# dotchen/LAV

Measured on NVIDIA H100. Metric: agent_frames_per_s, higher is better.
Workload: dtype fp16 storage, fp32 accumulate (wgmma f16 / mma.sync f16; saturating stores)

## Files before the change

### lav_b200/csrc/conv_pair_umma.cu

```cuda
#include <stdlib.h>
#include "sm90.cuh"

namespace lavb {
namespace pair {

constexpr int kBlockM = 128, kBlockK = 64;
constexpr int kABytes = kBlockM * kBlockK * 2;
constexpr int kMaxStages = 8;
constexpr int kPairThreads = 288;

struct PairArgs {
  int n, h, w, c, kchunks, dil, tile_w, tile_h, tiles_per_img, num_tiles, stages, post_relu;
  const h16* res;
  const float* bias1; const float* shift2;
  long long* trace; int trace_tiles;
};
#define PAIR_STAMP(slot, i)                                                                                         \
  do {                                                                                                              \
    if (p.trace && threadIdx.x == 0 && (i) < p.trace_tiles)                                                         \
      p.trace[((long long)blockIdx.x * p.trace_tiles + (i)) * 8 + (slot)] = clock64();                              \
  } while (0)

using namespace sm90;

__device__ __forceinline__ uint32_t relu2(uint32_t x) {
  const h162 v = __hmax2(*reinterpret_cast<const h162*>(&x), floats2h162(0.f, 0.f));
  return *reinterpret_cast<const uint32_t*>(&v);
}
__device__ __forceinline__ uint32_t add2(uint32_t x, uint32_t r, bool relu) {
  const h162 a = *reinterpret_cast<const h162*>(&x), b = *reinterpret_cast<const h162*>(&r);
  h162 v = relu ? __hfma2_relu(a, floats2h162(1.f, 1.f), b) : __hadd2(a, b);
#ifndef LAVB_H16_BF16
  const uint32_t hi = 0x7BFF7BFFu, lo = 0xFBFFFBFFu;
  v = __hmin2(v, *reinterpret_cast<const h162*>(&hi));
  if (!relu) v = __hmax2(v, *reinterpret_cast<const h162*>(&lo));
#endif
  return *reinterpret_cast<const uint32_t*>(&v);
}

template <int kC>
__global__ void __launch_bounds__(kPairThreads, kC == 64 ? 2 : 1) conv_pair_umma_kernel(const __grid_constant__ CUtensorMap tmap_a,
                                                                                       const __grid_constant__ CUtensorMap tmap_w1,
                                                                                       const __grid_constant__ CUtensorMap tmap_w2,
                                                                                       const __grid_constant__ CUtensorMap tmap_r,
                                                                                       const __grid_constant__ CUtensorMap tmap_o,
                                                                                       const __grid_constant__ PairArgs p) {
  constexpr int kNC = kC / 64;
  constexpr int kChunks = kC / kBlockK;
  constexpr int kWBytes = kC * kBlockK * 2;
  constexpr int kSlotBytes = kABytes + kWBytes;
  constexpr int kNkb = 3 * kChunks;
  constexpr int kBpf = kSlotBytes / kWBytes;
  constexpr int kOutBytes = kChunks * kABytes;
  static_assert(kNkb % kBpf == 0, "stage 2 fills whole ring slots");
  static_assert(kOutBytes <= kSlotBytes, "the residual / output tile fits one ring slot");
  extern __shared__ uint8_t smem_raw[];
  const uint32_t base = (smem_u32(smem_raw) + 1023u) & ~1023u;
  uint8_t* gen = smem_raw + (base - smem_u32(smem_raw));
  const uint32_t mid = base + p.stages * kSlotBytes;
  constexpr int kMidBytes = 3 * kChunks * kABytes;
  const uint32_t ctrl = mid + kMidBytes;
  const uint32_t full_bar = ctrl, empty_bar = ctrl + 8 * kMaxStages;
  float* ep_b1 = reinterpret_cast<float*>(gen + (ctrl - base) + 16 * kMaxStages);
  float* ep_t2 = ep_b1 + 128;

  const int warp = threadIdx.x >> 5, lane = threadIdx.x & 31;
  if (threadIdx.x == 0) {
    asm volatile("prefetch.tensormap [%0];" ::"l"(reinterpret_cast<uint64_t>(&tmap_a)) : "memory");
    asm volatile("prefetch.tensormap [%0];" ::"l"(reinterpret_cast<uint64_t>(&tmap_w1)) : "memory");
    asm volatile("prefetch.tensormap [%0];" ::"l"(reinterpret_cast<uint64_t>(&tmap_w2)) : "memory");
    asm volatile("prefetch.tensormap [%0];" ::"l"(reinterpret_cast<uint64_t>(&tmap_r)) : "memory");
    asm volatile("prefetch.tensormap [%0];" ::"l"(reinterpret_cast<uint64_t>(&tmap_o)) : "memory");
    for (int s = 0; s < p.stages; ++s) { mbar_init(full_bar + 8 * s, 1); mbar_init(empty_bar + 8 * s, 8); }
    asm volatile("fence.mbarrier_init.release.cluster;" ::: "memory");
  }
  for (int c = threadIdx.x; c < kC; c += blockDim.x) {
    ep_b1[c] = __ldg(p.bias1 + c);
    ep_t2[c] = p.shift2 ? __ldg(p.shift2 + c) : 0.f;
  }
  for (int i = threadIdx.x; i < kMidBytes / 16; i += blockDim.x)
    *reinterpret_cast<uint4*>(gen + (mid - base) + 16 * i) = make_uint4(0u, 0u, 0u, 0u);
  proxy_fence_async();
  __syncthreads();

  if (warp == 8) {
    if (lane == 0) {
      int slot = 0; uint32_t phase = 0;
      for (int tile = blockIdx.x; tile < p.num_tiles; tile += gridDim.x) {
        const int img = tile / p.tiles_per_img, y0 = (tile - img * p.tiles_per_img) * p.tile_h;
        for (int t = 0; t < 3; ++t)
          for (int kc = 0; kc < kChunks; ++kc) {
            mbar_wait(empty_bar + 8 * slot, phase ^ 1);
            const uint32_t sa = base + slot * kSlotBytes;
            mbar_expect_tx(full_bar + 8 * slot, kSlotBytes);
            tma_load_4d(sa, &tmap_a, full_bar + 8 * slot, kc * kBlockK, 0, y0 + (t - 1) * p.dil, img);
            tma_load_2d(sa + kABytes, &tmap_w1, full_bar + 8 * slot, kc * kBlockK, t * kC);
            if (++slot == p.stages) { slot = 0; phase ^= 1; }
          }
        for (int kb0 = 0; kb0 < kNkb; kb0 += kBpf) {
          mbar_wait(empty_bar + 8 * slot, phase ^ 1);
          const uint32_t sa = base + slot * kSlotBytes;
          mbar_expect_tx(full_bar + 8 * slot, kBpf * kWBytes);
          for (int b = 0; b < kBpf; ++b) {
            const int kb = kb0 + b, t = kb / kChunks, kc = kb - t * kChunks;
            tma_load_2d(sa + b * kWBytes, &tmap_w2, full_bar + 8 * slot, kc * kBlockK, t * kC);
          }
          if (++slot == p.stages) { slot = 0; phase ^= 1; }
        }
        mbar_wait(empty_bar + 8 * slot, phase ^ 1);
        if (p.res) {
          mbar_expect_tx(full_bar + 8 * slot, kOutBytes);
          for (int kc = 0; kc < kChunks; ++kc)
            tma_load_4d(base + slot * kSlotBytes + kc * kABytes, &tmap_r, full_bar + 8 * slot, kc * kBlockK, 0, y0, img);
        } else {
          mbar_arrive(full_bar + 8 * slot);
        }
        if (++slot == p.stages) { slot = 0; phase ^= 1; }
      }
    }
    return;
  }

  const int wg = warp >> 2;
  const int d = p.dil;
  const bool relu_out = p.post_relu != 0;
  uint8_t* midp = gen + (mid - base);
  int slot = 0; uint32_t phase = 0;
  int i = 0;
  for (int tile = blockIdx.x; tile < p.num_tiles; tile += gridDim.x, ++i) {
    const int img = tile / p.tiles_per_img, y0 = (tile - img * p.tiles_per_img) * p.tile_h;
    float acc[kC / 2];
    int prev = -1;
    for (int kb = 0; kb < kNkb; ++kb) {
      mbar_wait(full_bar + 8 * slot, phase);
      const uint32_t sa = base + slot * kSlotBytes;
      const uint64_t a_desc = sm90::desc_sw128(sa + wg * (kABytes / 2)), b_desc = sm90::desc_sw128(sa + kABytes);
      sm90::wgmma_fence();
#pragma unroll
      for (int k = 0; k < kBlockK / 16; ++k)
        sm90::wgmma<kC>(acc, a_desc + (uint64_t)(2 * k), b_desc + (uint64_t)(2 * k), (kb | k) ? 1u : 0u);
      sm90::wgmma_commit();
      sm90::wgmma_wait<1>();
      if (prev >= 0 && lane == 0) mbar_arrive(empty_bar + 8 * prev);
      prev = slot;
      if (++slot == p.stages) { slot = 0; phase ^= 1; }
    }
    sm90::wgmma_wait<0>();
    sm90::acc_fence(acc);
    if (lane == 0) mbar_arrive(empty_bar + 8 * prev);
    PAIR_STAMP(0, i);
    sm90::bar_sync(1, 256);
#pragma unroll
    for (int h = 0; h < 2; ++h) {
      const int m = 64 * wg + 16 * (warp & 3) + (lane >> 2) + 8 * h;
      const int px = m % p.tile_w;
      const bool ok0 = px + d < p.tile_w, ok2 = px - d >= 0;
      const int r0 = m + d, r2 = m - d;
#pragma unroll
      for (int cc = 0; cc < kNC; ++cc)
#pragma unroll
        for (int j = 0; j < 8; ++j) {
          const int col = 64 * cc + 8 * j + 2 * (lane & 3);
          const float2 b = *reinterpret_cast<const float2*>(ep_b1 + col);
          const uint32_t v = relu2(pack_h16(acc[32 * cc + 4 * j + 2 * h] + b.x, acc[32 * cc + 4 * j + 2 * h + 1] + b.y));
          uint8_t* blk = midp + cc * kABytes + (col & 7) * 2;
          if (ok0) *reinterpret_cast<uint32_t*>(blk + 0 * kChunks * kABytes + r0 * 128 + ((j ^ (r0 & 7)) << 4)) = v;
          *reinterpret_cast<uint32_t*>(blk + 1 * kChunks * kABytes + m * 128 + ((j ^ (m & 7)) << 4)) = v;
          if (ok2) *reinterpret_cast<uint32_t*>(blk + 2 * kChunks * kABytes + r2 * 128 + ((j ^ (r2 & 7)) << 4)) = v;
        }
    }
    proxy_fence_async();
    sm90::bar_sync(1, 256);
    PAIR_STAMP(1, i);
    prev = -1;
    for (int kb0 = 0; kb0 < kNkb; kb0 += kBpf) {
      mbar_wait(full_bar + 8 * slot, phase);
      const uint32_t sa = base + slot * kSlotBytes;
      sm90::wgmma_fence();
#pragma unroll
      for (int b = 0; b < kBpf; ++b) {
        const uint64_t a_desc = sm90::desc_sw128(mid + (kb0 + b) * kABytes + wg * (kABytes / 2)), b_desc = sm90::desc_sw128(sa + b * kWBytes);
#pragma unroll
        for (int k = 0; k < kBlockK / 16; ++k)
          sm90::wgmma<kC>(acc, a_desc + (uint64_t)(2 * k), b_desc + (uint64_t)(2 * k), (kb0 | b | k) ? 1u : 0u);
      }
      sm90::wgmma_commit();
      sm90::wgmma_wait<1>();
      if (prev >= 0 && lane == 0) mbar_arrive(empty_bar + 8 * prev);
      prev = slot;
      if (++slot == p.stages) { slot = 0; phase ^= 1; }
    }
    sm90::wgmma_wait<0>();
    sm90::acc_fence(acc);
    if (lane == 0) mbar_arrive(empty_bar + 8 * prev);
    PAIR_STAMP(2, i);
    const int out_slot = slot; const uint32_t out_phase = phase;
    if (++slot == p.stages) { slot = 0; phase ^= 1; }
    mbar_wait(full_bar + 8 * out_slot, out_phase);
    uint8_t* outp = gen + out_slot * kSlotBytes;
#pragma unroll
    for (int h = 0; h < 2; ++h) {
      const int m = 64 * wg + 16 * (warp & 3) + (lane >> 2) + 8 * h;
#pragma unroll
      for (int cc = 0; cc < kNC; ++cc)
#pragma unroll
        for (int j = 0; j < 8; ++j) {
          const int col = 64 * cc + 8 * j + 2 * (lane & 3);
          const float2 t = *reinterpret_cast<const float2*>(ep_t2 + col);
          uint32_t* o = reinterpret_cast<uint32_t*>(outp + cc * kABytes + m * 128 + ((j ^ (m & 7)) << 4) + (col & 7) * 2);
          uint32_t v = pack_h16(acc[32 * cc + 4 * j + 2 * h] + t.x, acc[32 * cc + 4 * j + 2 * h + 1] + t.y);
          if (p.res) v = add2(v, *o, relu_out);
          else if (relu_out) v = relu2(v);
          *o = v;
        }
    }
    proxy_fence_async();
    sm90::bar_sync(1, 256);
    if (threadIdx.x == 0) {
      for (int kc = 0; kc < kChunks; ++kc) tma_store_4d(&tmap_o, base + out_slot * kSlotBytes + kc * kABytes, kc * kBlockK, 0, y0, img);
      bulk_commit();
      bulk_wait_read<0>();
      mbar_arrive(empty_bar + 8 * out_slot, 8);
    }
    PAIR_STAMP(3, i);
  }
  if (threadIdx.x == 0) bulk_wait<0>();
}

}
}

using namespace lavb;
using namespace lavb::pair;

static long long* g_pair_trace = nullptr;
static int g_pair_trace_tiles = 0;
extern "C" int lavb_conv_pair_set_trace(void* d_buf, int tiles_per_cta) {
  g_pair_trace = reinterpret_cast<long long*>(d_buf);
  g_pair_trace_tiles = d_buf ? tiles_per_cta : 0;
  return 0;
}

extern "C" int lavb_conv_pair_umma(const lavb_conv_pair_desc* d, void* stream) {
  LAVB_CHECK_ARG(d != nullptr, "conv_pair_umma: null descriptor");
  LAVB_CHECK_ARG(d->c == 64 || d->c == 128, "conv_pair_umma: channels must be 64 or 128 (got %d)", d->c);
  LAVB_CHECK_ARG(d->w == 32 || d->w == 64 || d->w == 128, "conv_pair_umma: image width must be 32, 64 or 128 (a tile is made of full rows)");
  LAVB_CHECK_ARG(d->dil >= 1 && d->dil < d->w, "conv_pair_umma: dilation must be in [1, width)");
  LAVB_CHECK_ARG(d->n >= 0 && d->h >= 1, "conv_pair_umma: bad shape");
  LAVB_CHECK_ARG(d->w1 && d->w2 && d->bias1 && d->in && d->out, "conv_pair_umma: null operand");
  {
    const size_t bytes = (size_t)d->n * d->h * d->w * d->c * 2;
    const auto overlap = [&](const void* x) {
      const char *o = static_cast<const char*>(d->out), *q = static_cast<const char*>(x);
      return x && o < q + bytes && q < o + bytes;
    };
    LAVB_CHECK_ARG(!overlap(d->in) && !overlap(d->res), "conv_pair_umma: out must not overlap in or res");
  }
  if (d->n == 0) return 0;
  auto encode = get_encode();
  LAVB_CHECK_ARG(encode != nullptr, "conv_pair_umma: cuTensorMapEncodeTiled not available from the driver");
  PairArgs a;
  memset(&a, 0, sizeof(a));
  a.n = d->n; a.h = d->h; a.w = d->w; a.c = d->c; a.kchunks = d->c / kBlockK; a.dil = d->dil;
  a.tile_w = d->w; a.tile_h = kBlockM / d->w;
  a.tiles_per_img = ceil_div(d->h, a.tile_h);
  a.num_tiles = d->n * a.tiles_per_img;
  a.post_relu = d->post_relu;
  a.res = reinterpret_cast<const h16*>(d->res);
  a.bias1 = d->bias1; a.shift2 = d->shift2;
  a.trace = g_pair_trace; a.trace_tiles = g_pair_trace_tiles;
  const int slot_bytes = kABytes + d->c * kBlockK * 2;
  const int mid_bytes = 3 * a.kchunks * kABytes;
  const int ctrl_bytes = 1024  + 16 * kMaxStages + 2 * 128 * (int)sizeof(float);
  const bool two = d->c == 64;
  const int smem_cap = two ? 113 * 1024 : 227 * 1024;
  a.stages = min(kMaxStages, (smem_cap - mid_bytes - ctrl_bytes) / slot_bytes);
  const int smem = a.stages * slot_bytes + mid_bytes + ctrl_bytes;
  CUtensorMap tmap_a, tmap_w1, tmap_w2, tmap_r, tmap_o;
  const auto encode_act = [&](CUtensorMap* m, const void* ptr) {
    cuuint64_t dims[4] = {(cuuint64_t)d->c, (cuuint64_t)d->w, (cuuint64_t)d->h, (cuuint64_t)d->n};
    cuuint64_t strides[3] = {(cuuint64_t)d->c * 2, (cuuint64_t)d->w * d->c * 2, (cuuint64_t)d->h * d->w * d->c * 2};
    cuuint32_t box[4] = {(cuuint32_t)kBlockK, (cuuint32_t)a.tile_w, (cuuint32_t)a.tile_h, 1};
    cuuint32_t estr[4] = {1, 1, 1, 1};
    return encode(m, LAVB_TMAP_H16, 4, const_cast<void*>(ptr), dims, strides, box, estr, CU_TENSOR_MAP_INTERLEAVE_NONE,
                  CU_TENSOR_MAP_SWIZZLE_128B, CU_TENSOR_MAP_L2_PROMOTION_L2_256B, CU_TENSOR_MAP_FLOAT_OOB_FILL_NONE);
  };
  CUresult r = encode_act(&tmap_a, d->in);
  LAVB_CHECK_ARG(r == CUDA_SUCCESS, "conv_pair_umma: cuTensorMapEncodeTiled(in) failed with %d", (int)r);
  r = encode_act(&tmap_r, d->res ? d->res : d->in);
  LAVB_CHECK_ARG(r == CUDA_SUCCESS, "conv_pair_umma: cuTensorMapEncodeTiled(res) failed with %d", (int)r);
  r = encode_act(&tmap_o, d->out);
  LAVB_CHECK_ARG(r == CUDA_SUCCESS, "conv_pair_umma: cuTensorMapEncodeTiled(out) failed with %d", (int)r);
  for (int which = 0; which < 2; ++which) {
    cuuint64_t dims[2] = {(cuuint64_t)d->c, (cuuint64_t)3 * d->c};
    cuuint64_t strides[1] = {(cuuint64_t)d->c * 2};
    cuuint32_t box[2] = {(cuuint32_t)kBlockK, (cuuint32_t)d->c};
    cuuint32_t estr[2] = {1, 1};
    CUresult r = encode(which ? &tmap_w2 : &tmap_w1, LAVB_TMAP_H16, 2, const_cast<void*>(which ? d->w2 : d->w1), dims,
                        strides, box, estr, CU_TENSOR_MAP_INTERLEAVE_NONE, CU_TENSOR_MAP_SWIZZLE_128B, CU_TENSOR_MAP_L2_PROMOTION_L2_256B,
                        CU_TENSOR_MAP_FLOAT_OOB_FILL_NONE);
    LAVB_CHECK_ARG(r == CUDA_SUCCESS, "conv_pair_umma: cuTensorMapEncodeTiled(W%d) failed with %d", which + 1, (int)r);
  }
  if (two) {
    LAVB_CUDA_OK(ensure_dyn_smem((const void*)conv_pair_umma_kernel<64>, smem_cap));
    conv_pair_umma_kernel<64><<<min(a.num_tiles, 2 * kNumSMs), kPairThreads, smem, (cudaStream_t)stream>>>(tmap_a, tmap_w1, tmap_w2, tmap_r, tmap_o, a);
  } else {
    LAVB_CUDA_OK(ensure_dyn_smem((const void*)conv_pair_umma_kernel<128>, smem_cap));
    conv_pair_umma_kernel<128><<<min(a.num_tiles, kNumSMs), kPairThreads, smem, (cudaStream_t)stream>>>(tmap_a, tmap_w1, tmap_w2, tmap_r, tmap_o, a);
  }
  LAVB_LAUNCH_OK();
  return 0;
}
```

### lav_b200/csrc/sm90.cuh

```cuda
#pragma once
#include <cuda.h>
#include <cudaTypedefs.h>
#include "common.cuh"

namespace lavb {
namespace sm90 {

__device__ __forceinline__ uint32_t smem_u32(const void* p) { return (uint32_t)__cvta_generic_to_shared(p); }

__device__ __forceinline__ void proxy_fence_async() { asm volatile("fence.proxy.async.shared::cta;" ::: "memory"); }
__device__ __forceinline__ void bar_sync(int id, int threads) { asm volatile("bar.sync %0, %1;" ::"r"(id), "r"(threads) : "memory"); }

__device__ __forceinline__ void mbar_init(uint32_t bar, uint32_t count) {
  asm volatile("mbarrier.init.shared::cta.b64 [%0], %1;" ::"r"(bar), "r"(count));
}
__device__ __forceinline__ void mbar_expect_tx(uint32_t bar, uint32_t bytes) {
  asm volatile("mbarrier.arrive.expect_tx.shared::cta.b64 _, [%0], %1;" ::"r"(bar), "r"(bytes) : "memory");
}
__device__ __forceinline__ void mbar_arrive(uint32_t bar) {
  asm volatile("mbarrier.arrive.shared::cta.b64 _, [%0];" ::"r"(bar) : "memory");
}
__device__ __forceinline__ void mbar_wait(uint32_t bar, uint32_t parity) {
  uint32_t done;
  do {
    asm volatile(
        "{\n\t.reg .pred p;\n\t"
        "mbarrier.try_wait.parity.shared::cta.b64 p, [%1], %2;\n\t"
        "selp.u32 %0, 1, 0, p;\n\t}"
        : "=r"(done) : "r"(bar), "r"(parity) : "memory");
  } while (!done);
}
__device__ __forceinline__ void tma_load_4d(uint32_t dst, const CUtensorMap* map, uint32_t bar, int c0, int c1, int c2, int c3) {
  asm volatile(
      "cp.async.bulk.tensor.4d.shared::cluster.global.mbarrier::complete_tx::bytes [%0], [%1, {%3, %4, %5, %6}], [%2];"
      ::"r"(dst), "l"(reinterpret_cast<uint64_t>(map)), "r"(bar), "r"(c0), "r"(c1), "r"(c2), "r"(c3) : "memory");
}
__device__ __forceinline__ void tma_load_2d(uint32_t dst, const CUtensorMap* map, uint32_t bar, int c0, int c1) {
  asm volatile(
      "cp.async.bulk.tensor.2d.shared::cluster.global.mbarrier::complete_tx::bytes [%0], [%1, {%3, %4}], [%2];"
      ::"r"(dst), "l"(reinterpret_cast<uint64_t>(map)), "r"(bar), "r"(c0), "r"(c1) : "memory");
}
__device__ __forceinline__ void mbar_arrive(uint32_t bar, uint32_t count) {
  asm volatile("mbarrier.arrive.shared::cta.b64 _, [%0], %1;" ::"r"(bar), "r"(count) : "memory");
}

__device__ __forceinline__ void tma_store_4d(const CUtensorMap* map, uint32_t src, int c0, int c1, int c2, int c3) {
  asm volatile("cp.async.bulk.tensor.4d.global.shared::cta.bulk_group [%0, {%2, %3, %4, %5}], [%1];"
               ::"l"(reinterpret_cast<uint64_t>(map)), "r"(src), "r"(c0), "r"(c1), "r"(c2), "r"(c3) : "memory");
}
__device__ __forceinline__ void bulk_commit() { asm volatile("cp.async.bulk.commit_group;" ::: "memory"); }
template <int N> __device__ __forceinline__ void bulk_wait_read() { asm volatile("cp.async.bulk.wait_group.read %0;" ::"n"(N) : "memory"); }
template <int N> __device__ __forceinline__ void bulk_wait() { asm volatile("cp.async.bulk.wait_group %0;" ::"n"(N) : "memory"); }

inline PFN_cuTensorMapEncodeTiled_v12000 get_encode() {
  static PFN_cuTensorMapEncodeTiled_v12000 fn = nullptr;
  if (!fn) {
    void* p = nullptr;
    cudaDriverEntryPointQueryResult q;
    if (cudaGetDriverEntryPoint("cuTensorMapEncodeTiled", &p, cudaEnableDefault, &q) == cudaSuccess && q == cudaDriverEntryPointSuccess)
      fn = reinterpret_cast<PFN_cuTensorMapEncodeTiled_v12000>(p);
  }
  return fn;
}

__device__ __forceinline__ uint64_t desc_sw128(uint32_t saddr) {
  const uint32_t lo = ((saddr & 0x3FFFFu) >> 4) | (1u << 16);
  const uint32_t hi = (1024u >> 4) | (1u << 30);
  return (uint64_t)lo | ((uint64_t)hi << 32);
}

__device__ __forceinline__ void wgmma_fence() { asm volatile("wgmma.fence.sync.aligned;" ::: "memory"); }
__device__ __forceinline__ void wgmma_commit() { asm volatile("wgmma.commit_group.sync.aligned;" ::: "memory"); }
template <int N> __device__ __forceinline__ void wgmma_wait() { asm volatile("wgmma.wait_group.sync.aligned %0;" ::"n"(N) : "memory"); }
template <int N> __device__ __forceinline__ void acc_fence(float (&d)[N]) {
#pragma unroll
  for (int i = 0; i < N; ++i) asm volatile("" : "+f"(d[i])::"memory");
}

template <int N> __device__ void wgmma(float (&d)[N / 2], uint64_t a, uint64_t b, uint32_t accumulate);

#define LAVB_WG_R0 "%0, %1, %2, %3, %4, %5, %6, %7, %8, %9, %10, %11, %12, %13, %14, %15"
#define LAVB_WG_R1 "%16, %17, %18, %19, %20, %21, %22, %23, %24, %25, %26, %27, %28, %29, %30, %31"
#define LAVB_WG_R2 "%32, %33, %34, %35, %36, %37, %38, %39, %40, %41, %42, %43, %44, %45, %46, %47"
#define LAVB_WG_R3 "%48, %49, %50, %51, %52, %53, %54, %55, %56, %57, %58, %59, %60, %61, %62, %63"
#define LAVB_WG_R4 "%64, %65, %66, %67, %68, %69, %70, %71, %72, %73, %74, %75, %76, %77, %78, %79"
#define LAVB_WG_R5 "%80, %81, %82, %83, %84, %85, %86, %87, %88, %89, %90, %91, %92, %93, %94, %95"
#define LAVB_WG_R6 "%96, %97, %98, %99, %100, %101, %102, %103, %104, %105, %106, %107, %108, %109, %110, %111"
#define LAVB_WG_R7 "%112, %113, %114, %115, %116, %117, %118, %119, %120, %121, %122, %123, %124, %125, %126, %127"
#define LAVB_WG_D4(i) "+f"(d[i]), "+f"(d[i + 1]), "+f"(d[i + 2]), "+f"(d[i + 3])
#define LAVB_WG_D16(i) LAVB_WG_D4(i), LAVB_WG_D4(i + 4), LAVB_WG_D4(i + 8), LAVB_WG_D4(i + 12)
#define LAVB_WGMMA(N, REGS, IA, IB, IP, ...)                                                                         \
  template <> __device__ __forceinline__ void wgmma<N>(float (&d)[N / 2], uint64_t a, uint64_t b, uint32_t accumulate) { \
    asm volatile(                                                                                                      \
        "{\n\t.reg .pred p;\n\t"                                                                                       \
        "setp.ne.b32 p, %" #IP ", 0;\n\t"                                                                              \
        "wgmma.mma_async.sync.aligned.m64n" #N "k16.f32." LAVB_H16_PTX "." LAVB_H16_PTX " "                            \
        "{" REGS "}, %" #IA ", %" #IB ", p, 1, 1, 0, 0;\n\t}"                                                          \
        : __VA_ARGS__                                                                                                  \
        : "l"(a), "l"(b), "r"(accumulate));                                                                            \
  }
LAVB_WGMMA(32, LAVB_WG_R0, 16, 17, 18, LAVB_WG_D16(0))
LAVB_WGMMA(64, LAVB_WG_R0 ", " LAVB_WG_R1, 32, 33, 34, LAVB_WG_D16(0), LAVB_WG_D16(16))
LAVB_WGMMA(96, LAVB_WG_R0 ", " LAVB_WG_R1 ", " LAVB_WG_R2, 48, 49, 50, LAVB_WG_D16(0), LAVB_WG_D16(16), LAVB_WG_D16(32))
LAVB_WGMMA(128, LAVB_WG_R0 ", " LAVB_WG_R1 ", " LAVB_WG_R2 ", " LAVB_WG_R3, 64, 65, 66,
           LAVB_WG_D16(0), LAVB_WG_D16(16), LAVB_WG_D16(32), LAVB_WG_D16(48))
LAVB_WGMMA(160, LAVB_WG_R0 ", " LAVB_WG_R1 ", " LAVB_WG_R2 ", " LAVB_WG_R3 ", " LAVB_WG_R4, 80, 81, 82,
           LAVB_WG_D16(0), LAVB_WG_D16(16), LAVB_WG_D16(32), LAVB_WG_D16(48), LAVB_WG_D16(64))
LAVB_WGMMA(192, LAVB_WG_R0 ", " LAVB_WG_R1 ", " LAVB_WG_R2 ", " LAVB_WG_R3 ", " LAVB_WG_R4 ", " LAVB_WG_R5, 96, 97, 98,
           LAVB_WG_D16(0), LAVB_WG_D16(16), LAVB_WG_D16(32), LAVB_WG_D16(48), LAVB_WG_D16(64), LAVB_WG_D16(80))
LAVB_WGMMA(224, LAVB_WG_R0 ", " LAVB_WG_R1 ", " LAVB_WG_R2 ", " LAVB_WG_R3 ", " LAVB_WG_R4 ", " LAVB_WG_R5 ", " LAVB_WG_R6,
           112, 113, 114, LAVB_WG_D16(0), LAVB_WG_D16(16), LAVB_WG_D16(32), LAVB_WG_D16(48), LAVB_WG_D16(64), LAVB_WG_D16(80),
           LAVB_WG_D16(96))
LAVB_WGMMA(256, LAVB_WG_R0 ", " LAVB_WG_R1 ", " LAVB_WG_R2 ", " LAVB_WG_R3 ", " LAVB_WG_R4 ", " LAVB_WG_R5 ", " LAVB_WG_R6 ", " LAVB_WG_R7,
           128, 129, 130, LAVB_WG_D16(0), LAVB_WG_D16(16), LAVB_WG_D16(32), LAVB_WG_D16(48), LAVB_WG_D16(64), LAVB_WG_D16(80),
           LAVB_WG_D16(96), LAVB_WG_D16(112))
#undef LAVB_WGMMA
#undef LAVB_WG_D16
#undef LAVB_WG_D4
#undef LAVB_WG_R0
#undef LAVB_WG_R1
#undef LAVB_WG_R2
#undef LAVB_WG_R3
#undef LAVB_WG_R4
#undef LAVB_WG_R5
#undef LAVB_WG_R6
#undef LAVB_WG_R7

}
}
```

Before: 1962.

## Overlap next tile's stage-1 GEMM with epilogue in fused conv pair kernel

Restructures the fused two-conv kernel so consumers issue the next tile's stage-1 wgmmas while still running the current tile's stage-2 epilogue, using a second accumulator set. For C=64 both weight sets stay resident in shared memory instead of being streamed per tile. The output/residual tile moves to its own double-buffered region with separate barriers so TMA stores overlap. A full producer warpgroup with setmaxnreg register rebalancing is added, and C=64 drops from two CTAs per SM to one. Register pressure is higher, and the lost second CTA on C=64 reduces inter-CTA overlap.

```diff
diff --git a/lav_b200/csrc/conv_pair_umma.cu b/lav_b200/csrc/conv_pair_umma.cu
--- a/lav_b200/csrc/conv_pair_umma.cu
+++ b/lav_b200/csrc/conv_pair_umma.cu
@@ -7,10 +7,35 @@
 constexpr int kBlockM = 128, kBlockK = 64;
 constexpr int kABytes = kBlockM * kBlockK * 2;
 constexpr int kMaxStages = 8;
-constexpr int kPairThreads = 288;
+constexpr int kPairThreads = 384;
+constexpr int kProducerRegs = 40, kConsumerRegs = 232;
+constexpr int kSmemCap = 227 * 1024;
+
+template <int kC>
+struct Cfg {
+  static constexpr bool kResident = kC == 64;
+  static constexpr int kNC = kC / 64;
+  static constexpr int kChunks = kC / kBlockK;
+  static constexpr int kWBytes = kC * kBlockK * 2;
+  static constexpr int kSlotBytes = kABytes + (kResident ? 0 : kWBytes);
+  static constexpr int kNkb = 3 * kChunks;
+  static constexpr int kBpf = kSlotBytes / kWBytes;
+  static constexpr int kOutBytes = kChunks * kABytes;
+  static constexpr int kMidBytes = 3 * kChunks * kABytes;
+  static constexpr int kResBytes = kResident ? 2 * kNkb * kWBytes : 0;
+  static constexpr int kPieces = 2 * kNC;
+  static constexpr int kAhead = kNkb - kPieces;
+  static constexpr int kOutBufs = kC == 64 ? 2 : 1;
+  static constexpr int kCtrlBytes = 1024  + 16 * kMaxStages + 64 + 2 * 128 * (int)sizeof(float);
+  static constexpr int kFixedBytes = kOutBufs * kOutBytes + kMidBytes + kResBytes + kCtrlBytes;
+  static constexpr int kStages = (kSmemCap - kFixedBytes) / kSlotBytes < kMaxStages ? (kSmemCap - kFixedBytes) / kSlotBytes : kMaxStages;
+  static constexpr int kSmemBytes = kStages * kSlotBytes + kFixedBytes;
+  static_assert(kResident || kNkb % kBpf == 0, "stage 2 fills whole ring slots");
+  static_assert(kAhead >= 1 && kStages >= kAhead + 1, "the look-ahead keeps kAhead + 1 stage-1 K-blocks in the ring");
+};
 
 struct PairArgs {
-  int n, h, w, c, kchunks, dil, tile_w, tile_h, tiles_per_img, num_tiles, stages, post_relu;
+  int n, h, w, c, kchunks, dil, tile_w, tile_h, tiles_per_img, num_tiles, post_relu;
   const h16* res;
   const float* bias1; const float* shift2;
   long long* trace; int trace_tiles;
@@ -38,31 +63,220 @@
   return *reinterpret_cast<const uint32_t*>(&v);
 }
 
-template <int kC>
-__global__ void __launch_bounds__(kPairThreads, kC == 64 ? 2 : 1) conv_pair_umma_kernel(const __grid_constant__ CUtensorMap tmap_a,
-                                                                                       const __grid_constant__ CUtensorMap tmap_w1,
-                                                                                       const __grid_constant__ CUtensorMap tmap_w2,
-                                                                                       const __grid_constant__ CUtensorMap tmap_r,
-                                                                                       const __grid_constant__ CUtensorMap tmap_o,
-                                                                                       const __grid_constant__ PairArgs p) {
-  constexpr int kNC = kC / 64;
-  constexpr int kChunks = kC / kBlockK;
-  constexpr int kWBytes = kC * kBlockK * 2;
-  constexpr int kSlotBytes = kABytes + kWBytes;
-  constexpr int kNkb = 3 * kChunks;
-  constexpr int kBpf = kSlotBytes / kWBytes;
-  constexpr int kOutBytes = kChunks * kABytes;
-  static_assert(kNkb % kBpf == 0, "stage 2 fills whole ring slots");
-  static_assert(kOutBytes <= kSlotBytes, "the residual / output tile fits one ring slot");
+struct Smem {
+  uint32_t ring, out, mid, wres;
+  uint32_t full_bar, empty_bar;
+  uint32_t out_full, out_empty;
+  uint32_t w_full;
+  uint8_t* gen;
+  float *ep_b1, *ep_t2;
+};
+
+struct RingPos {
+  int slot = 0; uint32_t phase = 0;
+  template <int kStages> __device__ __forceinline__ void next() { if (++slot == kStages) { slot = 0; phase ^= 1; } }
+};
+
+struct Consumer {
+  RingPos head; int tail = 0;
+  int wg, warp, lane;
+  template <int kStages> __device__ __forceinline__ void release(const Smem& s) {
+    if (lane == 0) mbar_arrive(s.empty_bar + 8 * tail);
+    if (++tail == kStages) tail = 0;
+  }
+};
+
+template <int kC>
+__device__ __forceinline__ void fill_stage1(const Smem& s, RingPos& pos, const CUtensorMap* tmap_a, const CUtensorMap* tmap_w1,
+                                            const PairArgs& p, int tile) {
+  using C = Cfg<kC>;
+  const int img = tile / p.tiles_per_img, y0 = (tile - img * p.tiles_per_img) * p.tile_h;
+  for (int t = 0; t < 3; ++t)
+    for (int kc = 0; kc < C::kChunks; ++kc) {
+      mbar_wait(s.empty_bar + 8 * pos.slot, pos.phase ^ 1);
+      const uint32_t sa = s.ring + pos.slot * C::kSlotBytes, bar = s.full_bar + 8 * pos.slot;
+      mbar_expect_tx(bar, C::kSlotBytes);
+      tma_load_4d(sa, tmap_a, bar, kc * kBlockK, 0, y0 + (t - 1) * p.dil, img);
+      if (!C::kResident) tma_load_2d(sa + kABytes, tmap_w1, bar, kc * kBlockK, t * kC);
+      pos.template next<C::kStages>();
+    }
+}
+
+template <int kC>
+__device__ __forceinline__ void issue_stage1(float (&acc1)[kC / 2], const Smem& s, Consumer& c, int kb) {
+  using C = Cfg<kC>;
+  mbar_wait(s.full_bar + 8 * c.head.slot, c.head.phase);
+  const uint32_t sa = s.ring + c.head.slot * C::kSlotBytes;
+  const uint64_t a_desc = desc_sw128(sa + c.wg * (kABytes / 2));
+  const uint64_t b_desc = desc_sw128(C::kResident ? s.wres + kb * C::kWBytes : sa + kABytes);
+  wgmma_fence();
+#pragma unroll
+  for (int k = 0; k < kBlockK / 16; ++k)
+    wgmma<kC>(acc1, a_desc + (uint64_t)(2 * k), b_desc + (uint64_t)(2 * k), (kb | k) ? 1u : 0u);
+  wgmma_commit();
+  c.head.template next<C::kStages>();
+}
+
+template <int kC>
+__device__ __forceinline__ void stage1(float (&acc1)[kC / 2], const Smem& s, Consumer& c) {
+  using C = Cfg<kC>;
+#pragma unroll
+  for (int kb = 0; kb < C::kNkb; ++kb) {
+    issue_stage1<kC>(acc1, s, c, kb);
+    wgmma_wait<1>();
+    if (kb) c.template release<C::kStages>(s);
+  }
+  wgmma_wait<0>();
+  acc_fence(acc1);
+  c.template release<C::kStages>(s);
+}
+
+template <int kC, bool kLook>
+__device__ __forceinline__ void finish_tile(float (&acc1)[kC / 2], float (&acc2)[kC / 2], const Smem& s, Consumer& c,
+                                            const CUtensorMap* tmap_o, const PairArgs& p, int tile, int i) {
+  using C = Cfg<kC>;
+  const int wg = c.wg, warp = c.warp, lane = c.lane, d = p.dil;
+  const bool relu_out = p.post_relu != 0;
+  const int img = tile / p.tiles_per_img, y0 = (tile - img * p.tiles_per_img) * p.tile_h;
+  uint8_t* midp = s.gen + (s.mid - s.ring);
+  bar_sync(1, 256);
+#pragma unroll
+  for (int h = 0; h < 2; ++h) {
+    const int m = 64 * wg + 16 * (warp & 3) + (lane >> 2) + 8 * h;
+    const int px = m % p.tile_w;
+    const bool ok0 = px + d < p.tile_w, ok2 = px - d >= 0;
+    const int r0 = m + d, r2 = m - d;
+#pragma unroll
+    for (int cc = 0; cc < C::kNC; ++cc) {
+      float2 b1v[8];
+#pragma unroll
+      for (int j = 0; j < 8; ++j) b1v[j] = *reinterpret_cast<const float2*>(s.ep_b1 + 64 * cc + 8 * j + 2 * (lane & 3));
+#pragma unroll
+      for (int j = 0; j < 8; ++j) {
+        const int col = 64 * cc + 8 * j + 2 * (lane & 3);
+        const float2 b = b1v[j];
+        const uint32_t v = relu2(pack_h16(acc1[32 * cc + 4 * j + 2 * h] + b.x, acc1[32 * cc + 4 * j + 2 * h + 1] + b.y));
+        uint8_t* blk = midp + cc * kABytes + (col & 7) * 2;
+        if (ok0) *reinterpret_cast<uint32_t*>(blk + 0 * C::kChunks * kABytes + r0 * 128 + ((j ^ (r0 & 7)) << 4)) = v;
+        *reinterpret_cast<uint32_t*>(blk + 1 * C::kChunks * kABytes + m * 128 + ((j ^ (m & 7)) << 4)) = v;
+        if (ok2) *reinterpret_cast<uint32_t*>(blk + 2 * C::kChunks * kABytes + r2 * 128 + ((j ^ (r2 & 7)) << 4)) = v;
+      }
+    }
+  }
+  proxy_fence_async();
+  bar_sync(1, 256);
+  PAIR_STAMP(1, i);
+  if (C::kResident) {
+    wgmma_fence();
+#pragma unroll
+    for (int kb = 0; kb < C::kNkb; ++kb) {
+      const uint64_t a_desc = desc_sw128(s.mid + kb * kABytes + wg * (kABytes / 2));
+      const uint64_t b_desc = desc_sw128(s.wres + (C::kNkb + kb) * C::kWBytes);
+#pragma unroll
+      for (int k = 0; k < kBlockK / 16; ++k)
+        wgmma<kC>(acc2, a_desc + (uint64_t)(2 * k), b_desc + (uint64_t)(2 * k), (kb | k) ? 1u : 0u);
+    }
+    wgmma_commit();
+  } else {
+#pragma unroll
+    for (int kb0 = 0; kb0 < C::kNkb; kb0 += C::kBpf) {
+      mbar_wait(s.full_bar + 8 * c.head.slot, c.head.phase);
+      const uint32_t sa = s.ring + c.head.slot * C::kSlotBytes;
+      wgmma_fence();
+#pragma unroll
+      for (int b = 0; b < C::kBpf; ++b) {
+        const uint64_t a_desc = desc_sw128(s.mid + (kb0 + b) * kABytes + wg * (kABytes / 2)), b_desc = desc_sw128(sa + b * C::kWBytes);
+#pragma unroll
+        for (int k = 0; k < kBlockK / 16; ++k)
+          wgmma<kC>(acc2, a_desc + (uint64_t)(2 * k), b_desc + (uint64_t)(2 * k), (kb0 | b | k) ? 1u : 0u);
+      }
+      wgmma_commit();
+      c.head.template next<C::kStages>();
+      wgmma_wait<1>();
+      if (kb0) c.template release<C::kStages>(s);
+    }
+  }
+  wgmma_wait<0>();
+  acc_fence(acc2);
+  if (!C::kResident) c.template release<C::kStages>(s);
+  PAIR_STAMP(2, i);
+  if (kLook) {
+#pragma unroll
+    for (int kb = 0; kb < C::kAhead; ++kb) issue_stage1<kC>(acc1, s, c, kb);
+    PAIR_STAMP(4, i);
+  }
+  const int ob = i % C::kOutBufs;
+  mbar_wait(s.out_full + 8 * ob, (i / C::kOutBufs) & 1);
+  uint8_t* outp = s.gen + (s.out - s.ring) + ob * C::kOutBytes;
+#pragma unroll
+  for (int h = 0; h < 2; ++h) {
+    const int m = 64 * wg + 16 * (warp & 3) + (lane >> 2) + 8 * h;
+#pragma unroll
+    for (int cc = 0; cc < C::kNC; ++cc) {
+      uint8_t* orow = outp + cc * kABytes + m * 128 + 4 * (lane & 3);
+      float2 t2v[8];
+      uint32_t r[8];
+#pragma unroll
+      for (int j = 0; j < 8; ++j) t2v[j] = *reinterpret_cast<const float2*>(s.ep_t2 + 64 * cc + 8 * j + 2 * (lane & 3));
+      if (p.res) {
+#pragma unroll
+        for (int j = 0; j < 8; ++j) r[j] = *reinterpret_cast<const uint32_t*>(orow + ((j ^ (m & 7)) << 4));
+      }
+#pragma unroll
+      for (int j = 0; j < 8; ++j) {
+        const float2 t = t2v[j];
+        uint32_t v = pack_h16(acc2[32 * cc + 4 * j + 2 * h] + t.x, acc2[32 * cc + 4 * j + 2 * h + 1] + t.y);
+        if (p.res) v = add2(v, r[j], relu_out);
+        else if (relu_out) v = relu2(v);
+        *reinterpret_cast<uint32_t*>(orow + ((j ^ (m & 7)) << 4)) = v;
+      }
+      if (kLook) {
+        issue_stage1<kC>(acc1, s, c, C::kAhead + h * C::kNC + cc);
+        wgmma_wait<C::kAhead>();
+        c.template release<C::kStages>(s);
+      }
+    }
+  }
+  if (kLook) PAIR_STAMP(5, i);
+  proxy_fence_async();
+  bar_sync(1, 256);
+  if (threadIdx.x == 0) {
+    for (int kc = 0; kc < C::kChunks; ++kc)
+      tma_store_4d(tmap_o, s.out + ob * C::kOutBytes + kc * kABytes, kc * kBlockK, 0, y0, img);
+    bulk_commit();
+    bulk_wait_read<C::kOutBufs - 1>();
+    if (i >= C::kOutBufs - 1) mbar_arrive(s.out_empty + 8 * ((i - (C::kOutBufs - 1)) % C::kOutBufs));
+  }
+  PAIR_STAMP(3, i);
+  if (kLook) {
+    wgmma_wait<0>();
+    acc_fence(acc1);
+#pragma unroll
+    for (int kb = 0; kb < C::kAhead; ++kb) c.template release<C::kStages>(s);
+    PAIR_STAMP(0, i + 1);
+  }
+}
+
+template <int kC>
+__global__ void __launch_bounds__(kPairThreads, 1) conv_pair_umma_kernel(const __grid_constant__ CUtensorMap tmap_a,
+                                                                         const __grid_constant__ CUtensorMap tmap_w1,
+                                                                         const __grid_constant__ CUtensorMap tmap_w2,
+                                                                         const __grid_constant__ CUtensorMap tmap_r,
+                                                                         const __grid_constant__ CUtensorMap tmap_o,
+                                                                         const __grid_constant__ PairArgs p) {
+  using C = Cfg<kC>;
   extern __shared__ uint8_t smem_raw[];
-  const uint32_t base = (smem_u32(smem_raw) + 1023u) & ~1023u;
-  uint8_t* gen = smem_raw + (base - smem_u32(smem_raw));
-  const uint32_t mid = base + p.stages * kSlotBytes;
-  constexpr int kMidBytes = 3 * kChunks * kABytes;
-  const uint32_t ctrl = mid + kMidBytes;
-  const uint32_t full_bar = ctrl, empty_bar = ctrl + 8 * kMaxStages;
-  float* ep_b1 = reinterpret_cast<float*>(gen + (ctrl - base) + 16 * kMaxStages);
-  float* ep_t2 = ep_b1 + 128;
+  Smem s;
+  s.ring = (smem_u32(smem_raw) + 1023u) & ~1023u;
+  s.gen = smem_raw + (s.ring - smem_u32(smem_raw));
+  s.out = s.ring + C::kStages * C::kSlotBytes;
+  s.mid = s.out + C::kOutBufs * C::kOutBytes;
+  s.wres = s.mid + C::kMidBytes;
+  const uint32_t ctrl = s.wres + C::kResBytes;
+  s.full_bar = ctrl; s.empty_bar = ctrl + 8 * kMaxStages;
+  s.out_full = ctrl + 16 * kMaxStages; s.out_empty = s.out_full + 16; s.w_full = s.out_full + 32;
+  s.ep_b1 = reinterpret_cast<float*>(s.gen + (ctrl - s.ring) + 16 * kMaxStages + 64);
+  s.ep_t2 = s.ep_b1 + 128;
 
   const int warp = threadIdx.x >> 5, lane = threadIdx.x & 31;
   if (threadIdx.x == 0) {
@@ -71,159 +285,74 @@
     asm volatile("prefetch.tensormap [%0];" ::"l"(reinterpret_cast<uint64_t>(&tmap_w2)) : "memory");
     asm volatile("prefetch.tensormap [%0];" ::"l"(reinterpret_cast<uint64_t>(&tmap_r)) : "memory");
     asm volatile("prefetch.tensormap [%0];" ::"l"(reinterpret_cast<uint64_t>(&tmap_o)) : "memory");
-    for (int s = 0; s < p.stages; ++s) { mbar_init(full_bar + 8 * s, 1); mbar_init(empty_bar + 8 * s, 8); }
+    for (int i = 0; i < C::kStages; ++i) { mbar_init(s.full_bar + 8 * i, 1); mbar_init(s.empty_bar + 8 * i, 8); }
+    for (int i = 0; i < C::kOutBufs; ++i) { mbar_init(s.out_full + 8 * i, 1); mbar_init(s.out_empty + 8 * i, 1); }
+    mbar_init(s.w_full, 1);
     asm volatile("fence.mbarrier_init.release.cluster;" ::: "memory");
   }
   for (int c = threadIdx.x; c < kC; c += blockDim.x) {
-    ep_b1[c] = __ldg(p.bias1 + c);
-    ep_t2[c] = p.shift2 ? __ldg(p.shift2 + c) : 0.f;
-  }
-  for (int i = threadIdx.x; i < kMidBytes / 16; i += blockDim.x)
-    *reinterpret_cast<uint4*>(gen + (mid - base) + 16 * i) = make_uint4(0u, 0u, 0u, 0u);
+    s.ep_b1[c] = __ldg(p.bias1 + c);
+    s.ep_t2[c] = p.shift2 ? __ldg(p.shift2 + c) : 0.f;
+  }
+  for (int i = threadIdx.x; i < C::kMidBytes / 16; i += blockDim.x)
+    *reinterpret_cast<uint4*>(s.gen + (s.mid - s.ring) + 16 * i) = make_uint4(0u, 0u, 0u, 0u);
   proxy_fence_async();
   __syncthreads();
 
-  if (warp == 8) {
-    if (lane == 0) {
-      int slot = 0; uint32_t phase = 0;
-      for (int tile = blockIdx.x; tile < p.num_tiles; tile += gridDim.x) {
+  const int first = blockIdx.x, step = gridDim.x;
+  if (warp >= 8) {
+    reg_dec<kProducerRegs>();
+    if (warp == 8 && lane == 0 && first < p.num_tiles) {
+      RingPos pos;
+      if (C::kResident) {
+        mbar_expect_tx(s.w_full, C::kResBytes);
+        for (int kb = 0; kb < 2 * C::kNkb; ++kb) {
+          const int t = (kb % C::kNkb) / C::kChunks, kc = kb % C::kChunks;
+          tma_load_2d(s.wres + kb * C::kWBytes, kb < C::kNkb ? &tmap_w1 : &tmap_w2, s.w_full, kc * kBlockK, t * kC);
+        }
+      }
+      fill_stage1<kC>(s, pos, &tmap_a, &tmap_w1, p, first);
+      int i = 0;
+      for (int tile = first; tile < p.num_tiles; tile += step, ++i) {
         const int img = tile / p.tiles_per_img, y0 = (tile - img * p.tiles_per_img) * p.tile_h;
-        for (int t = 0; t < 3; ++t)
-          for (int kc = 0; kc < kChunks; ++kc) {
-            mbar_wait(empty_bar + 8 * slot, phase ^ 1);
-            const uint32_t sa = base + slot * kSlotBytes;
-            mbar_expect_tx(full_bar + 8 * slot, kSlotBytes);
-            tma_load_4d(sa, &tmap_a, full_bar + 8 * slot, kc * kBlockK, 0, y0 + (t - 1) * p.dil, img);
-            tma_load_2d(sa + kABytes, &tmap_w1, full_bar + 8 * slot, kc * kBlockK, t * kC);
-            if (++slot == p.stages) { slot = 0; phase ^= 1; }
+        if (!C::kResident)
+          for (int kb0 = 0; kb0 < C::kNkb; kb0 += C::kBpf) {
+            mbar_wait(s.empty_bar + 8 * pos.slot, pos.phase ^ 1);
+            const uint32_t sa = s.ring + pos.slot * C::kSlotBytes, bar = s.full_bar + 8 * pos.slot;
+            mbar_expect_tx(bar, C::kBpf * C::kWBytes);
+            for (int b = 0; b < C::kBpf; ++b) {
+              const int kb = kb0 + b, t = kb / C::kChunks, kc = kb - t * C::kChunks;
+              tma_load_2d(sa + b * C::kWBytes, &tmap_w2, bar, kc * kBlockK, t * kC);
+            }
+            pos.template next<C::kStages>();
           }
-        for (int kb0 = 0; kb0 < kNkb; kb0 += kBpf) {
-          mbar_wait(empty_bar + 8 * slot, phase ^ 1);
-          const uint32_t sa = base + slot * kSlotBytes;
-          mbar_expect_tx(full_bar + 8 * slot, kBpf * kWBytes);
-          for (int b = 0; b < kBpf; ++b) {
-            const int kb = kb0 + b, t = kb / kChunks, kc = kb - t * kChunks;
-            tma_load_2d(sa + b * kWBytes, &tmap_w2, full_bar + 8 * slot, kc * kBlockK, t * kC);
-          }
-          if (++slot == p.stages) { slot = 0; phase ^= 1; }
+        const int ob = i % C::kOutBufs;
+        const uint32_t out_bar = s.out_full + 8 * ob;
+        mbar_wait(s.out_empty + 8 * ob, ((i / C::kOutBufs) & 1) ^ 1);
+        if (p.res) {
+          mbar_expect_tx(out_bar, C::kOutBytes);
+          for (int kc = 0; kc < C::kChunks; ++kc)
+            tma_load_4d(s.out + ob * C::kOutBytes + kc * kABytes, &tmap_r, out_bar, kc * kBlockK, 0, y0, img);
+        } else {
+          mbar_arrive(out_bar);
         }
-        mbar_wait(empty_bar + 8 * slot, phase ^ 1);
-        if (p.res) {
-          mbar_expect_tx(full_bar + 8 * slot, kOutBytes);
-          for (int kc = 0; kc < kChunks; ++kc)
-            tma_load_4d(base + slot * kSlotBytes + kc * kABytes, &tmap_r, full_bar + 8 * slot, kc * kBlockK, 0, y0, img);
-        } else {
-          mbar_arrive(full_bar + 8 * slot);
-        }
-        if (++slot == p.stages) { slot = 0; phase ^= 1; }
+        if (tile + step < p.num_tiles) fill_stage1<kC>(s, pos, &tmap_a, &tmap_w1, p, tile + step);
       }
     }
     return;
   }
 
-  const int wg = warp >> 2;
-  const int d = p.dil;
-  const bool relu_out = p.post_relu != 0;
-  uint8_t* midp = gen + (mid - base);
-  int slot = 0; uint32_t phase = 0;
-  int i = 0;
-  for (int tile = blockIdx.x; tile < p.num_tiles; tile += gridDim.x, ++i) {
-    const int img = tile / p.tiles_per_img, y0 = (tile - img * p.tiles_per_img) * p.tile_h;
-    float acc[kC / 2];
-    int prev = -1;
-    for (int kb = 0; kb < kNkb; ++kb) {
-      mbar_wait(full_bar + 8 * slot, phase);
-      const uint32_t sa = base + slot * kSlotBytes;
-      const uint64_t a_desc = sm90::desc_sw128(sa + wg * (kABytes / 2)), b_desc = sm90::desc_sw128(sa + kABytes);
-      sm90::wgmma_fence();
-#pragma unroll
-      for (int k = 0; k < kBlockK / 16; ++k)
-        sm90::wgmma<kC>(acc, a_desc + (uint64_t)(2 * k), b_desc + (uint64_t)(2 * k), (kb | k) ? 1u : 0u);
-      sm90::wgmma_commit();
-      sm90::wgmma_wait<1>();
-      if (prev >= 0 && lane == 0) mbar_arrive(empty_bar + 8 * prev);
-      prev = slot;
-      if (++slot == p.stages) { slot = 0; phase ^= 1; }
-    }
-    sm90::wgmma_wait<0>();
-    sm90::acc_fence(acc);
-    if (lane == 0) mbar_arrive(empty_bar + 8 * prev);
-    PAIR_STAMP(0, i);
-    sm90::bar_sync(1, 256);
-#pragma unroll
-    for (int h = 0; h < 2; ++h) {
-      const int m = 64 * wg + 16 * (warp & 3) + (lane >> 2) + 8 * h;
-      const int px = m % p.tile_w;
-      const bool ok0 = px + d < p.tile_w, ok2 = px - d >= 0;
-      const int r0 = m + d, r2 = m - d;
-#pragma unroll
-      for (int cc = 0; cc < kNC; ++cc)
-#pragma unroll
-        for (int j = 0; j < 8; ++j) {
-          const int col = 64 * cc + 8 * j + 2 * (lane & 3);
-          const float2 b = *reinterpret_cast<const float2*>(ep_b1 + col);
-          const uint32_t v = relu2(pack_h16(acc[32 * cc + 4 * j + 2 * h] + b.x, acc[32 * cc + 4 * j + 2 * h + 1] + b.y));
-          uint8_t* blk = midp + cc * kABytes + (col & 7) * 2;
-          if (ok0) *reinterpret_cast<uint32_t*>(blk + 0 * kChunks * kABytes + r0 * 128 + ((j ^ (r0 & 7)) << 4)) = v;
-          *reinterpret_cast<uint32_t*>(blk + 1 * kChunks * kABytes + m * 128 + ((j ^ (m & 7)) << 4)) = v;
-          if (ok2) *reinterpret_cast<uint32_t*>(blk + 2 * kChunks * kABytes + r2 * 128 + ((j ^ (r2 & 7)) << 4)) = v;
-        }
-    }
-    proxy_fence_async();
-    sm90::bar_sync(1, 256);
-    PAIR_STAMP(1, i);
-    prev = -1;
-    for (int kb0 = 0; kb0 < kNkb; kb0 += kBpf) {
-      mbar_wait(full_bar + 8 * slot, phase);
-      const uint32_t sa = base + slot * kSlotBytes;
-      sm90::wgmma_fence();
-#pragma unroll
-      for (int b = 0; b < kBpf; ++b) {
-        const uint64_t a_desc = sm90::desc_sw128(mid + (kb0 + b) * kABytes + wg * (kABytes / 2)), b_desc = sm90::desc_sw128(sa + b * kWBytes);
-#pragma unroll
-        for (int k = 0; k < kBlockK / 16; ++k)
-          sm90::wgmma<kC>(acc, a_desc + (uint64_t)(2 * k), b_desc + (uint64_t)(2 * k), (kb0 | b | k) ? 1u : 0u);
-      }
-      sm90::wgmma_commit();
-      sm90::wgmma_wait<1>();
-      if (prev >= 0 && lane == 0) mbar_arrive(empty_bar + 8 * prev);
-      prev = slot;
-      if (++slot == p.stages) { slot = 0; phase ^= 1; }
-    }
-    sm90::wgmma_wait<0>();
-    sm90::acc_fence(acc);
-    if (lane == 0) mbar_arrive(empty_bar + 8 * prev);
-    PAIR_STAMP(2, i);
-    const int out_slot = slot; const uint32_t out_phase = phase;
-    if (++slot == p.stages) { slot = 0; phase ^= 1; }
-    mbar_wait(full_bar + 8 * out_slot, out_phase);
-    uint8_t* outp = gen + out_slot * kSlotBytes;
-#pragma unroll
-    for (int h = 0; h < 2; ++h) {
-      const int m = 64 * wg + 16 * (warp & 3) + (lane >> 2) + 8 * h;
-#pragma unroll
-      for (int cc = 0; cc < kNC; ++cc)
-#pragma unroll
-        for (int j = 0; j < 8; ++j) {
-          const int col = 64 * cc + 8 * j + 2 * (lane & 3);
-          const float2 t = *reinterpret_cast<const float2*>(ep_t2 + col);
-          uint32_t* o = reinterpret_cast<uint32_t*>(outp + cc * kABytes + m * 128 + ((j ^ (m & 7)) << 4) + (col & 7) * 2);
-          uint32_t v = pack_h16(acc[32 * cc + 4 * j + 2 * h] + t.x, acc[32 * cc + 4 * j + 2 * h + 1] + t.y);
-          if (p.res) v = add2(v, *o, relu_out);
-          else if (relu_out) v = relu2(v);
-          *o = v;
-        }
-    }
-    proxy_fence_async();
-    sm90::bar_sync(1, 256);
-    if (threadIdx.x == 0) {
-      for (int kc = 0; kc < kChunks; ++kc) tma_store_4d(&tmap_o, base + out_slot * kSlotBytes + kc * kABytes, kc * kBlockK, 0, y0, img);
-      bulk_commit();
-      bulk_wait_read<0>();
-      mbar_arrive(empty_bar + 8 * out_slot, 8);
-    }
-    PAIR_STAMP(3, i);
-  }
+  reg_inc<kConsumerRegs>();
+  if (first >= p.num_tiles) return;
+  Consumer c;
+  c.wg = warp >> 2; c.warp = warp; c.lane = lane;
+  float acc1[kC / 2], acc2[kC / 2];
+  if (C::kResident) mbar_wait(s.w_full, 0);
+  stage1<kC>(acc1, s, c);
+  PAIR_STAMP(0, 0);
+  int tile = first, i = 0;
+  for (; tile + step < p.num_tiles; tile += step, ++i) finish_tile<kC, true>(acc1, acc2, s, c, &tmap_o, p, tile, i);
+  finish_tile<kC, false>(acc1, acc2, s, c, &tmap_o, p, tile, i);
   if (threadIdx.x == 0) bulk_wait<0>();
 }
 
@@ -239,6 +368,15 @@
   g_pair_trace = reinterpret_cast<long long*>(d_buf);
   g_pair_trace_tiles = d_buf ? tiles_per_cta : 0;
   return 0;
+}
+
+template <int kC>
+static cudaError_t launch_pair(const CUtensorMap& tmap_a, const CUtensorMap& tmap_w1, const CUtensorMap& tmap_w2, const CUtensorMap& tmap_r,
+                               const CUtensorMap& tmap_o, const PairArgs& a, cudaStream_t stream) {
+  const cudaError_t e = ensure_dyn_smem((const void*)conv_pair_umma_kernel<kC>, Cfg<kC>::kSmemBytes);
+  if (e != cudaSuccess) return e;
+  conv_pair_umma_kernel<kC><<<min(a.num_tiles, kNumSMs), kPairThreads, Cfg<kC>::kSmemBytes, stream>>>(tmap_a, tmap_w1, tmap_w2, tmap_r, tmap_o, a);
+  return cudaSuccess;
 }
 
 extern "C" int lavb_conv_pair_umma(const lavb_conv_pair_desc* d, void* stream) {
@@ -269,13 +407,6 @@
   a.res = reinterpret_cast<const h16*>(d->res);
   a.bias1 = d->bias1; a.shift2 = d->shift2;
   a.trace = g_pair_trace; a.trace_tiles = g_pair_trace_tiles;
-  const int slot_bytes = kABytes + d->c * kBlockK * 2;
-  const int mid_bytes = 3 * a.kchunks * kABytes;
-  const int ctrl_bytes = 1024  + 16 * kMaxStages + 2 * 128 * (int)sizeof(float);
-  const bool two = d->c == 64;
-  const int smem_cap = two ? 113 * 1024 : 227 * 1024;
-  a.stages = min(kMaxStages, (smem_cap - mid_bytes - ctrl_bytes) / slot_bytes);
-  const int smem = a.stages * slot_bytes + mid_bytes + ctrl_bytes;
   CUtensorMap tmap_a, tmap_w1, tmap_w2, tmap_r, tmap_o;
   const auto encode_act = [&](CUtensorMap* m, const void* ptr) {
     cuuint64_t dims[4] = {(cuuint64_t)d->c, (cuuint64_t)d->w, (cuuint64_t)d->h, (cuuint64_t)d->n};
@@ -301,13 +432,8 @@
                         CU_TENSOR_MAP_FLOAT_OOB_FILL_NONE);
     LAVB_CHECK_ARG(r == CUDA_SUCCESS, "conv_pair_umma: cuTensorMapEncodeTiled(W%d) failed with %d", which + 1, (int)r);
   }
-  if (two) {
-    LAVB_CUDA_OK(ensure_dyn_smem((const void*)conv_pair_umma_kernel<64>, smem_cap));
-    conv_pair_umma_kernel<64><<<min(a.num_tiles, 2 * kNumSMs), kPairThreads, smem, (cudaStream_t)stream>>>(tmap_a, tmap_w1, tmap_w2, tmap_r, tmap_o, a);
-  } else {
-    LAVB_CUDA_OK(ensure_dyn_smem((const void*)conv_pair_umma_kernel<128>, smem_cap));
-    conv_pair_umma_kernel<128><<<min(a.num_tiles, kNumSMs), kPairThreads, smem, (cudaStream_t)stream>>>(tmap_a, tmap_w1, tmap_w2, tmap_r, tmap_o, a);
-  }
+  LAVB_CUDA_OK(d->c == 64 ? launch_pair<64>(tmap_a, tmap_w1, tmap_w2, tmap_r, tmap_o, a, (cudaStream_t)stream)
+                          : launch_pair<128>(tmap_a, tmap_w1, tmap_w2, tmap_r, tmap_o, a, (cudaStream_t)stream));
   LAVB_LAUNCH_OK();
   return 0;
 }
diff --git a/lav_b200/csrc/sm90.cuh b/lav_b200/csrc/sm90.cuh
--- a/lav_b200/csrc/sm90.cuh
+++ b/lav_b200/csrc/sm90.cuh
@@ -10,6 +10,9 @@
 
 __device__ __forceinline__ void proxy_fence_async() { asm volatile("fence.proxy.async.shared::cta;" ::: "memory"); }
 __device__ __forceinline__ void bar_sync(int id, int threads) { asm volatile("bar.sync %0, %1;" ::"r"(id), "r"(threads) : "memory"); }
+
+template <int N> __device__ __forceinline__ void reg_dec() { asm volatile("setmaxnreg.dec.sync.aligned.u32 %0;" ::"n"(N)); }
+template <int N> __device__ __forceinline__ void reg_inc() { asm volatile("setmaxnreg.inc.sync.aligned.u32 %0;" ::"n"(N)); }
 
 __device__ __forceinline__ void mbar_init(uint32_t bar, uint32_t count) {
   asm volatile("mbarrier.init.shared::cta.b64 [%0], %1;" ::"r"(bar), "r"(count));
```

Result: no change. 1964, median of 6 (+0.1%).
